# Jhuighuy/StormRuler

Measured on AMD Instinct MI355X. Metric: CG iterations/sec, 256^3 Poisson per GPU (+ SpMV achieved HBM GB/s in `roofline`), higher is better.
Workload: dtype f64

## Files before the change

stormruler_amd/csrc/common.hpp:

```cpp
#pragma once

#include <hip/hip_runtime.h>

#include <cstdint>
#include <cstdio>
#include <string>
#include <unordered_map>
#include <vector>

#include "../../include/storm_hip.h"

namespace storm {

void set_error(const char *fmt, ...) __attribute__((format(printf, 1, 2)));

#define STORM_FAIL(code, ...)        \
  do {                               \
    ::storm::set_error(__VA_ARGS__); \
    return (code);                   \
  } while (0)

#define STORM_REQUIRE(cond, ...) \
  do {                           \
    if (!(cond)) STORM_FAIL(STORM_HIP_E_INVALID, __VA_ARGS__); \
// ... 95 lines not shown
    int k = 0;
    bool ready = false;
    double value[storm::kMaxMulti] = {};
  } result_ring[storm::kResultRing];
  storm::SolverState *d_state = nullptr;
  storm::SolverState *h_state = nullptr;
  unsigned long long *h_done_ring = nullptr;
  unsigned long long *d_done_ring = nullptr;
  std::vector<storm::KrylovRes> krylov_free;
  unsigned long long ring_gen = 0;
  int64_t opt_ell_cap = 0;
  int64_t opt_spmv_dict = 4;
  int64_t opt_spmv_spw = 0;
  int64_t opt_spmv_xcd_remap = 8;
  int64_t opt_spmv_xcd_remap_sell = 64;
  int64_t opt_nt = 1;
  int stream_reverse = 0;
  int spmv_reverse = 0;
  int64_t opt_spmv_canon_tile_min_rows = (int64_t)1 << 20;
  int64_t opt_spmv_record_index = 1;
  int64_t opt_spmv_canon_tile = 2;
  int64_t opt_mgs_steps = 4;
  int64_t opt_resident_early = 1;
  int64_t opt_resident_apply_cache = 1;
  int64_t opt_resident_halo_interleave = 1;
  int64_t opt_coop_mgs_prefetch = 1;
  int64_t opt_coop_mgs_lds_prefetch = 1;
  int64_t opt_coop_mgs_rotate_early = 1;
  int64_t opt_coop_mgs_alternate = 1;
  int64_t opt_coop_mgs_xcd_runs = 1;
  int64_t opt_coop_mgs_apply = 1;
  int64_t opt_coop_mgs_quad = 1;
  char *d_quad_slots = nullptr;
  int64_t opt_coop_mgs_lds = 1;
  int64_t opt_spmv_mixed = 1;
  int64_t opt_profile_spmv = 0;
  std::vector<storm::LazyStmt> lazy_q;
  std::unordered_map<const void *, int> occupancy;
  int64_t opt_test_disable = 0;
  int64_t opt_lazy = 0;
  int callback_depth = 0;
  int64_t n_lazy_fused_dots = 0, n_lazy_fused_pairs = 0, n_lazy_apply_dots = 0, n_lazy_cg_steps = 0;
  storm_hip_vec *lazy_spare = nullptr;
  int64_t opt_profile_comm = 0;
  int64_t opt_blas1_nt = 1;
  int64_t opt_coop_mgs = 1;
  int64_t opt_latency_publish = 1;
  int64_t opt_coop_plain = 1;
  int64_t opt_coop_force_fail = 0;
  int coop_ran = 0;
  int coop_disabled = 0;
  int coop_fallback = 0;
  int64_t coop_skip = 0, coop_backoff = 0;
  int64_t opt_latency_path = 1;
  int64_t opt_resident_path = 1;
  int64_t opt_resident_max_rows = (int64_t)1 << 22;
  int64_t opt_resident_planes = 0;
  char *d_res_exch = nullptr;
  int64_t res_exch_rows = 0;
  int64_t opt_resident_profile = 0;
  long long *d_res_prof = nullptr;
  int res_prof_blocks = 0;
  char *d_res_slots = nullptr;
  int opt_lin_fuse = 1;
  int64_t opt_ticket_verify_inject = 0;
  int64_t opt_ticket_verify = 0;
  int opt_ticket_reduce = 1;
  int opt_fused_reduce = 1;
  int opt_latency_cache = 1;
  int64_t opt_latency_rows = 1 << 19;
  int64_t opt_rccl_fused = 1;
  int64_t opt_rccl_ticket = 1;
  int64_t opt_comm_wait_seconds = 120;
  int64_t opt_rccl_flag_wait = 1;
  int64_t opt_rccl_early_halo = 1;
  int64_t opt_generic_solvers = 0;
  int64_t opt_cg_march_fill = 2048;
  int64_t opt_cg_march_alternate = 1;
  int64_t opt_cg_march = 8;
  int64_t opt_cg_residual_march = 1;
  int64_t opt_cg_residual_planes = 1;
  int64_t opt_cg_residual_chunk = 16;
  int64_t opt_cg_residual_fill = 512;
  int64_t opt_cg_fuse = 1;
  std::vector<std::pair<size_t, double *>> pool;
  struct VecArena {
    char *base = nullptr;
    size_t bytes = 0, pitch = 0;
    int slots = 0, used = 0;
  };
  std::vector<VecArena> arenas;
  int64_t opt_vec_arena = 1;
  size_t pool_bytes = 0;
  int64_t opt_pool_bytes = (int64_t)16 << 30;
  std::vector<hipEvent_t> prof_events;
  size_t prof_used = 0;
  const int *api_done = nullptr;
  int64_t n_resident_solves = 0, n_latency_solves = 0, n_throughput_solves = 0, n_engine_solves = 0, n_cg_fused_steps = 0;
  int64_t n_block_solves = 0;
  int64_t n_cg_residual_marches = 0;
  int64_t n_cg_residual_plane_marches = 0;
  int64_t n_mgs_chain_steps = 0, n_mgs_quad_steps = 0;
  storm::Comm *comm = nullptr;
  int n_ranks = 1, rank = 0;
};

struct storm_hip_vec {
  storm_hip_ctx *ctx = nullptr;
  int64_t n_owned = 0, n_halo = 0;
  double *d = nullptr;
  double *base = nullptr;
  size_t bytes = 0;
  bool exposed = false;
};
constexpr int kVecGuard = 32;

namespace storm {

struct HaloPlan {
  int n_nbrs = 0;
  std::vector<int> nbr_rank;
  std::vector<int64_t> send_ptr, recv_ptr;
  int *d_send_idx = nullptr;
  double *d_sendbuf = nullptr;
  int64_t n_send = 0;
};

}

struct storm_hip_op {
  storm_hip_ctx *ctx = nullptr;
  int64_t n_rows = 0, n_halo = 0;
  int64_t n_slices = 0, n_interior_slices = 0;
  int64_t nnz = 0, ell_slots = 0, max_row_len = 0;
  int64_t *d_slice_off = nullptr;
  char *d_pack = nullptr;
  double *d_dict = nullptr;
  int dict_size = 0;
  int *d_offs = nullptr;
  int offs_size = 0;
  int xcd_group_sell = 0;
  int pair = 0;
  uint8_t *d_rec_idx = nullptr;
  uint64_t *d_rec_words = nullptr;
  int rec_words = 0;
  char *d_bnd_pack = nullptr;
  int bnd_width = 0;
  int canon_k = 0, canon_m1 = -1;
  int canon_off[7] = {0, 0, 0, 0, 0, 0, 0};
  int64_t pack_bytes = 0;
  int64_t spw = 1;
  int64_t tail_rows = 0, tail_nnz = 0;
  int *d_tail_row = nullptr;
  int64_t *d_tail_ptr = nullptr;
  int *d_tail_col = nullptr;
  double *d_tail_val = nullptr;
  int uniform_width = 0;
  std::vector<int> h_interior, h_boundary;
  int *d_interior = nullptr, *d_boundary = nullptr;
  int64_t n_interior = 0, n_boundary = 0;
  int64_t int_plane0 = 0, int_plane1 = 0;
  int64_t device_bytes = 0;
  char *d_lat_pack = nullptr;
  int64_t *d_lat_off = nullptr;
  int64_t lat_bytes = 0;
  storm::HaloPlan halo;
};

namespace storm {

struct Scal {
  const double *p;
  double v;
  double sign;
};
static inline Scal host_scal(double v) { return Scal{nullptr, v, 1.0}; }
static inline Scal dev_scal(const double *p, double sign = 1.0) { return Scal{p, 0.0, sign}; }

constexpr int kUnroll = 4;
constexpr int kStreamBlockElems = kBlock * kUnroll * 2;
constexpr int kMaxStreamBlocks = 32768;
static inline int stream_blocks(int64_t n) {
  int64_t b = (n + kStreamBlockElems - 1) / kStreamBlockElems;
  if (b < 1) b = 1;
// ... 136 lines not shown
```

stormruler_amd/csrc/context.hip:

```cpp
#include <cstdarg>
#include <cstring>
#include <random>

#include <algorithm>
#include "common.hpp"

#include <cstddef>

namespace storm {

static thread_local char g_error[1024] = "";

void set_error(const char *fmt, ...) {
  va_list ap;
  va_start(ap, fmt);
  vsnprintf(g_error, sizeof g_error, fmt, ap);
  va_end(ap);
}

}

using namespace storm;

static void pool_release(storm_hip_ctx *c);
// ... 110 lines not shown
    strncpy(name, c->name.c_str(), (size_t)name_len - 1);
    name[name_len - 1] = 0;
  }
  if (num_cus) *num_cus = c->num_cus;
  if (total_mem_bytes) *total_mem_bytes = c->total_mem;
  return STORM_HIP_OK;
}

int storm_hip_ctx_set_option(storm_hip_ctx *c, const char *key, int64_t value) {
  STORM_REQUIRE(c && key, "ctx_set_option: null argument");
  if (!strcmp(key, "ell_cap")) c->opt_ell_cap = value;
  else if (!strcmp(key, "generic_solvers")) c->opt_generic_solvers = value;
  else if (!strcmp(key, "rccl_fused")) c->opt_rccl_fused = value;
  else if (!strcmp(key, "rccl_ticket")) c->opt_rccl_ticket = value;
  else if (!strcmp(key, "rccl_early_halo")) c->opt_rccl_early_halo = value;
  else if (!strcmp(key, "rccl_flag_wait")) c->opt_rccl_flag_wait = value;
  else if (!strcmp(key, "comm_wait_seconds")) {
    STORM_REQUIRE(value >= 1 && value <= 3600, "ctx_set_option: comm_wait_seconds %lld (1 .. 3600)", (long long)value);
    c->opt_comm_wait_seconds = value;
  }
  else if (!strcmp(key, "latency_path")) c->opt_latency_path = value;
  else if (!strcmp(key, "resident_path")) c->opt_resident_path = value;
  else if (!strcmp(key, "resident_max_rows")) c->opt_resident_max_rows = value;
  else if (!strcmp(key, "resident_planes")) c->opt_resident_planes = value;
  else if (!strcmp(key, "resident_profile")) c->opt_resident_profile = value;
  else if (!strcmp(key, "coop_force_fail")) c->opt_coop_force_fail = value;
  else if (!strcmp(key, "coop_mgs")) c->opt_coop_mgs = value;
  else if (!strcmp(key, "coop_mgs_lds")) c->opt_coop_mgs_lds = value;
  else if (!strcmp(key, "coop_mgs_quad")) c->opt_coop_mgs_quad = value;
  else if (!strcmp(key, "cg_march_fill")) c->opt_cg_march_fill = value;
  else if (!strcmp(key, "resident_early")) c->opt_resident_early = value;
  else if (!strcmp(key, "mgs_steps")) c->opt_mgs_steps = value;
  else if (!strcmp(key, "vec_arena")) c->opt_vec_arena = value;
  else if (!strcmp(key, "spmv_mixed")) c->opt_spmv_mixed = value;
  else if (!strcmp(key, "spmv_canon_tile")) c->opt_spmv_canon_tile = value;
  else if (!strcmp(key, "spmv_canon_tile_min_rows")) c->opt_spmv_canon_tile_min_rows = value;
  else if (!strcmp(key, "fused_reduce")) c->opt_fused_reduce = (int)value;
  else if (!strcmp(key, "ticket_reduce")) c->opt_ticket_reduce = (int)value;
  else if (!strcmp(key, "ticket_verify")) c->opt_ticket_verify = value;
  else if (!strcmp(key, "ticket_verify_inject")) c->opt_ticket_verify_inject = value;
  else if (!strcmp(key, "lin_fuse")) c->opt_lin_fuse = (int)value;
  else if (!strcmp(key, "latency_rows")) c->opt_latency_rows = value;
  else if (!strcmp(key, "latency_cache")) c->opt_latency_cache = (int)value;
  else if (!strcmp(key, "nontemporal")) c->opt_nt = value;
  else if (!strcmp(key, "spmv_dict")) c->opt_spmv_dict = value;
  else if (!strcmp(key, "pool_bytes")) {
    c->opt_pool_bytes = value;
    if ((int64_t)c->pool_bytes > value || (value == 0 && !c->pool.empty())) {
      (void)hipStreamSynchronize(c->stream);
      pool_release(c);
    }
  }
  else if (!strcmp(key, "spmv_spw")) c->opt_spmv_spw = value;
  else if (!strcmp(key, "spmv_xcd_remap")) {
    STORM_REQUIRE(value >= 0 && value <= 4096, "ctx_set_option: spmv_xcd_remap %lld (0 .. 4096)", (long long)value);
    c->opt_spmv_xcd_remap = c->opt_spmv_xcd_remap_sell = value;
  }
  else if (!strcmp(key, "test_disable")) {
    c->opt_test_disable = value;
    c->opt_coop_mgs_apply = !(value & 1), c->opt_coop_mgs_prefetch = c->opt_coop_mgs_lds_prefetch = !(value & 2);
    c->opt_resident_apply_cache = !(value & 4), c->opt_resident_halo_interleave = !(value & 8);
    c->opt_latency_publish = !(value & 16), c->opt_coop_plain = !(value & 32), c->opt_cg_march_alternate = !(value & 64);
    c->opt_coop_mgs_xcd_runs = !(value & 128), c->opt_coop_mgs_alternate = !(value & 256);
    c->opt_coop_mgs_rotate_early = !(value & 512);
  }
  else if (!strcmp(key, "lazy_statements")) {
    if (value == 0) {
      STORM_TRY(lazy_sync(c));
      if (c->lazy_spare) (void)storm_hip_vec_destroy(c->lazy_spare), c->lazy_spare = nullptr;
    }
    c->opt_lazy = value;
  }
  else if (!strcmp(key, "profile_spmv")) c->opt_profile_spmv = value;
  else if (!strcmp(key, "profile_comm")) {
    c->opt_profile_comm = value;
    if (value != 0) STORM_TRY(comm_profile_reset(c));
  }
  else if (!strcmp(key, "cg_fuse")) c->opt_cg_fuse = value;
  else if (!strcmp(key, "cg_march")) c->opt_cg_march = value;
  else if (!strcmp(key, "cg_residual_march")) c->opt_cg_residual_march = value;
  else if (!strcmp(key, "cg_residual_planes")) c->opt_cg_residual_planes = value;
  else if (!strcmp(key, "cg_residual_chunk")) c->opt_cg_residual_chunk = value;
  else if (!strcmp(key, "cg_residual_fill")) c->opt_cg_residual_fill = value;
  else if (!strcmp(key, "spmv_record_index")) c->opt_spmv_record_index = value;
  else if (!strcmp(key, "blas1_nt")) c->opt_blas1_nt = value;
  else STORM_FAIL(STORM_HIP_E_INVALID, "ctx_set_option: unknown key '%s'", key);
  return STORM_HIP_OK;
}

int storm_hip_ctx_get_counter(storm_hip_ctx *c, const char *key, int64_t *value) {
  STORM_REQUIRE(c && key && value, "ctx_get_counter: null argument");
  if (!strcmp(key, "resident_solves")) *value = c->n_resident_solves;
  else if (!strcmp(key, "latency_solves")) *value = c->n_latency_solves;
  else if (!strcmp(key, "throughput_solves")) *value = c->n_throughput_solves;
  else if (!strcmp(key, "engine_solves")) *value = c->n_engine_solves;
  else if (!strcmp(key, "block_solves")) *value = c->n_block_solves;
  else if (!strcmp(key, "cg_fused_steps")) *value = c->n_cg_fused_steps;
  else if (!strcmp(key, "cg_residual_marches")) *value = c->n_cg_residual_marches;
  else if (!strcmp(key, "cg_residual_plane_marches")) *value = c->n_cg_residual_plane_marches;
  else if (!strcmp(key, "mgs_chain_steps")) *value = c->n_mgs_chain_steps;
  else if (!strcmp(key, "mgs_quad_steps")) *value = c->n_mgs_quad_steps;
  else if (!strcmp(key, "lazy_fused_dots")) *value = c->n_lazy_fused_dots;
  else if (!strcmp(key, "lazy_fused_pairs")) *value = c->n_lazy_fused_pairs;
  else if (!strcmp(key, "lazy_apply_dots")) *value = c->n_lazy_apply_dots;
  else if (!strcmp(key, "lazy_cg_steps")) *value = c->n_lazy_cg_steps;
  else if (!strcmp(key, "lazy_waiting")) *value = (int64_t)c->lazy_q.size();
  else if (!strncmp(key, "ipc_", 4)) {
    static const char *names[6] = {"ipc_allreduce_wait_ticks", "ipc_allreduces", "ipc_ack_wait_ticks", "ipc_ack_waits",
                                   "ipc_halo_slow_poll_ticks", "ipc_halo_slow_polls"};
    int k = -1;
    for (int i = 0; i < 6; ++i)
      if (!strcmp(key, names[i])) k = i;
    STORM_REQUIRE(k >= 0, "ctx_get_counter: unknown key '%s'", key);
    const long long v = comm_ipc_stat(c, k);
    STORM_REQUIRE(v >= 0, "ctx_get_counter: '%s' needs the peer-window transport", key);
    *value = v;
  }
  else if (!strncmp(key, "rccl_prof_", 10)) {
    static const char *names[8] = {"rccl_prof_exchanges", "rccl_prof_event_to_comm_ticks", "rccl_prof_pack_ticks",
                                   "rccl_prof_sendrecv_ticks", "rccl_prof_unhidden_wait_ticks", "rccl_prof_resume_ticks",
                                   "rccl_prof_allreduces", "rccl_prof_allreduce_ticks"};
    int k = -1;
    for (int i = 0; i < 8; ++i)
      if (!strcmp(key, names[i])) k = i;
    STORM_REQUIRE(k >= 0, "ctx_get_counter: unknown key '%s'", key);
    const long long v = comm_profile_read(c, k);
    STORM_REQUIRE(v >= 0, "ctx_get_counter: '%s' needs the RCCL transport with option profile_comm = 1", key);
    *value = v;
  }
  else if (!strncmp(key, "resident_phase_max_", 19) || !strncmp(key, "resident_phase_mean_", 20)) {
    const bool mx = key[15] == 'm' && key[16] == 'a';
    const int k = atoi(key + (mx ? 19 : 20));
    STORM_REQUIRE(c->d_res_prof != nullptr && c->res_prof_blocks > 0 && k >= 0 && k < 8, "ctx_get_counter: no resident profile (option resident_profile)");
    std::vector<long long> h((size_t)c->res_prof_blocks * 8);
    HIP_TRY(hipStreamSynchronize(c->stream));
    HIP_TRY(hipMemcpy(h.data(), c->d_res_prof, sizeof(long long) * h.size(), hipMemcpyDeviceToHost));
    long long m = 0, sum = 0;
    for (int b = 0; b < c->res_prof_blocks; ++b) m = std::max(m, h[(size_t)b * 8 + k]), sum += h[(size_t)b * 8 + k];
    *value = mx ? m : sum / c->res_prof_blocks;
  } else if (!strncmp(key, "resident_phase_block_", 21)) {
    int b = 0, k = 0;
    STORM_REQUIRE(sscanf(key + 21, "%d_%d", &b, &k) == 2 && c->d_res_prof != nullptr && b >= 0 && b < c->res_prof_blocks && k >= 0 && k < 8,
                  "ctx_get_counter: no such block / phase");
    long long v = 0;
    HIP_TRY(hipStreamSynchronize(c->stream));
    HIP_TRY(hipMemcpy(&v, c->d_res_prof + (size_t)b * 8 + k, sizeof v, hipMemcpyDeviceToHost));
    *value = v;
  }
  else STORM_FAIL(STORM_HIP_E_INVALID, "ctx_get_counter: unknown key '%s'", key);
  return STORM_HIP_OK;
}

int storm_hip_ctx_get_spmv_profile(storm_hip_ctx *c, int64_t *launches, double *total_ms, double *min_ms) {
  STORM_REQUIRE(c, "get_spmv_profile: null context");
  HIP_TRY(hipStreamSynchronize(c->stream));
  double total = 0.0, mn = 0.0;
  const size_t pairs = c->prof_used / 2;
  for (size_t i = 0; i < pairs; ++i) {
    float ms = 0.f;
    HIP_TRY(hipEventElapsedTime(&ms, c->prof_events[2 * i], c->prof_events[2 * i + 1]));
    total += ms;
    if (i == 0 || ms < mn) mn = ms;
  }
  if (launches) *launches = (int64_t)pairs;
  if (total_ms) *total_ms = total;
  if (min_ms) *min_ms = mn;
  c->prof_used = 0;
  return STORM_HIP_OK;
}

int storm_hip_ctx_get_spmv_profile_samples(storm_hip_ctx *c, double *ms_out, int64_t capacity, int64_t *count) {
  STORM_REQUIRE(c && count && (ms_out || capacity == 0), "get_spmv_profile_samples: null argument");
  HIP_TRY(hipStreamSynchronize(c->stream));
  const size_t pairs = c->prof_used / 2;
  for (size_t i = 0; i < pairs && (int64_t)i < capacity; ++i) {
    float ms = 0.f;
    HIP_TRY(hipEventElapsedTime(&ms, c->prof_events[2 * i], c->prof_events[2 * i + 1]));
    ms_out[i] = ms;
  }
  *count = (int64_t)pairs;
  c->prof_used = 0;
  return STORM_HIP_OK;
// ... 354 lines not shown
```

stormruler_amd/csrc/solver_cg.hip:

```cpp
#include <algorithm>
#include "solver_fused.hpp"
#include "blas1_device.hpp"
#include "spmv_device.hpp"

namespace storm {

__device__ __forceinline__ double cg_r_alpha(SolverState *st, const double *__restrict__ pz_partials, int n_pz, double *lds4) {
  double pz;
  if (pz_partials) {
    pz = block_fold(pz_partials, n_pz, lds4);
    if (blockIdx.x == 0 && threadIdx.x == 0) st->s[S_PZ] = pz;
  } else {
    pz = st->s[S_PZ];
  }
  const double alpha = safe_divide(st->s[S_GAMMA], pz);
  if (blockIdx.x == 0 && threadIdx.x == 0) st->s[S_ALPHA] = alpha;
  return alpha;
}
__device__ __forceinline__ void cg_r_finish(SolverState *st, double acc, unsigned bx, double *__restrict__ partials,
                                            const TicketArgs &tickets, const IpcDev &w, int use_ipc, double *lds4) {
  const double s = block_sum256(acc, lds4);
  if (tickets.cnt == nullptr) {
    if (threadIdx.x == 0) partials[bx] = s;
    return;
  }
  if (threadIdx.x >= kWave) return;
  const double mine[1] = {s};
  double total[1];
  if (ticket_reduce_wave0<1>(tickets, mine, 1, bx, gridDim.x, total)) {
    if (use_ipc == 1) ipc_allreduce_wave<1>(w, total, 1);
    if (threadIdx.x == 0) {
      st->s[S_GAMMA_NEW] = total[0];
      if (use_ipc != 2) do_step(STEP_CG_RR, st, GmresDev{});
    }
  }
}

__global__ __launch_bounds__(kBlock) void cg_r_kernel(int64_t n, SolverState *st, double *__restrict__ r,
                                                      const double *__restrict__ z,
                                                      double *__restrict__ partials, int nt,
                                                      const double *__restrict__ pz_partials, int n_pz, int reverse,
                                                      TicketArgs tickets, IpcDev w, int use_ipc) {
  if (st->done) return;
  __shared__ double lds4[4];
  const unsigned bx = reverse ? gridDim.x - 1 - blockIdx.x : blockIdx.x;
  const double alpha = cg_r_alpha(st, pz_partials, n_pz, lds4);
  double acc = 0.0;
  const int64_t n2 = n >> 1;
  double2v *r2 = reinterpret_cast<double2v *>(r);
  const double2v *z2 = reinterpret_cast<const double2v *>(z);
  nt_dispatch(nt, [&](auto nt) {
  for (int64_t base = (int64_t)bx * (kBlock * kUnroll) + threadIdx.x; base < n2;
       base += (int64_t)gridDim.x * (kBlock * kUnroll)) {
    double2v vr[kUnroll], vz[kUnroll];
#pragma unroll
    for (int u = 0; u < kUnroll; ++u) {
      const int64_t i = base + u * kBlock;
      if (i < n2) vr[u] = ldv(r2 + i, nt), vz[u] = ldv(z2 + i, nt);
    }
#pragma unroll
    for (int u = 0; u < kUnroll; ++u) {
      const int64_t i = base + u * kBlock;
      if (i < n2) {
        vr[u] -= alpha * vz[u];
        stv(r2 + i, vr[u], nt);
        acc += vr[u].x * vr[u].x;
        acc += vr[u].y * vr[u].y;
      }
    }
  }
  });
  if ((n & 1) && bx == 0 && threadIdx.x == 0) {
    const double vr = r[n - 1] - alpha * z[n - 1];
    r[n - 1] = vr;
    acc += vr * vr;
  }
  cg_r_finish(st, acc, bx, partials, tickets, w, use_ipc, lds4);
}

template <bool IDX>
__global__ __launch_bounds__(kBlock) void cg_r_recompute_kernel(int64_t n, SolverState *st, double *__restrict__ r,
                                                                const double *__restrict__ p, SellArgs A, CanonTileArgs T,
                                                                Scal alpha_s, Scal beta_s, const double *__restrict__ pz_partials,
                                                                int n_pz, int reverse, TicketArgs tickets) {
  if (st->done) return;
  __shared__ double lds4[4];
  __shared__ double dict_sh[32];
  extern __shared__ __attribute__((aligned(16))) unsigned long long words_sh[];
  const int lane = threadIdx.x & (kWave - 1);
  if (threadIdx.x < 32) dict_sh[threadIdx.x] = A.dict[threadIdx.x];
  if (IDX) rec_table_fill(A, words_sh);
  __syncthreads();
  const unsigned bx = reverse ? gridDim.x - 1 - blockIdx.x : blockIdx.x;
  const double alpha = cg_r_alpha(st, pz_partials, n_pz, lds4);
  const double op_alpha = ld_scal2(alpha_s), op_beta = ld_scal2(beta_s);
  const int64_t a = T.a, b = T.b, mg = T.max_gather;
  const char *pg = reinterpret_cast<const char *>(p) - (size_t)kVecGuard * 8;
  auto pair_at = [&](int64_t row) {
    int64_t gi = row + kVecGuard;
    gi = gi < 0 ? 0 : (gi > mg ? mg : gi);
// ... 8 lines not shown
  const int64_t n2 = n >> 1;
  double2v *r2 = reinterpret_cast<double2v *>(r);
  for (int64_t base = (int64_t)bx * (kBlock * kUnroll) + threadIdx.x; base - lane < n2;
       base += (int64_t)gridDim.x * (kBlock * kUnroll)) {
    double2v vr[kUnroll], c[kUnroll], nb[kUnroll][4];
    double el[kUnroll];
    RecRaw<IDX> w[kUnroll];
#pragma unroll
    for (int u = 0; u < kUnroll; ++u) {
      const int64_t i = base + u * kBlock;
      const int64_t row = 2 * (i < n2 ? i : n2 - 1);
      vr[u] = r2[row >> 1];
      c[u] = pair_at(row);
      w[u] = rec_load<IDX>(A, (uint32_t)row);
      nb[u][0] = pair_at(row - b), nb[u][1] = pair_at(row - a), nb[u][2] = pair_at(row + a), nb[u][3] = pair_at(row + b);
      el[u] = 0.0;
      if (lane == 0) el[u] = one_at(row - 1);
      if (lane == kWave - 1) el[u] = one_at(row + 2);
    }
#pragma unroll
    for (int u = 0; u < kUnroll; ++u) {
      const int64_t i = base + u * kBlock;
      double2v xg[6];
      xg[0] = nb[u][0], xg[1] = nb[u][1], xg[4] = nb[u][2], xg[5] = nb[u][3];
      const double left = dpp_shift<0x138>(c[u].y);
      const double right = dpp_shift<0x130>(c[u].x);
      xg[2].x = lane == 0 ? el[u] : left;
      xg[2].y = c[u].x;
      xg[3].x = c[u].y;
      xg[3].y = lane == kWave - 1 ? el[u] : right;
      const double2v vz = lattice_pair_apply(dict_sh, rec_word<IDX>(w[u], words_sh), xg, c[u], op_alpha, op_beta);
      if (i < n2) {
        vr[u] -= alpha * vz;
        r2[i] = vr[u];
        acc += vr[u].x * vr[u].x;
        acc += vr[u].y * vr[u].y;
      }
    }
  }
  cg_r_finish(st, acc, bx, nullptr, tickets, IpcDev{}, 0, lds4);
}

static bool cg_r_recompute_applies(const storm_hip_op *op, bool tick) {
  storm_hip_ctx *c = op->ctx;
  MarchArgs M;
  int nb = 0;
  return c->opt_cg_residual_march != 0 && tick && c->comm == nullptr && c->opt_ticket_verify == 0 && op->n_rows % 2 == 0 &&
         spmv_can_march(op) && cg_march_geometry(op, &M, &nb);
}
static int cg_r_recompute_run(const storm_hip_op *op, int nbv, Scal alpha, Scal beta, const double *p, SolverState *st, double *r,
                              const double *pz_partials, int n_pz, int reverse) {
  storm_hip_ctx *c = op->ctx;
  CanonTileArgs T;
  int nbt = 0;
  STORM_REQUIRE(canon_tile_geometry(op, &T, &nbt), "cg: the residual recompute needs a lattice operator");
  const SellArgs A = lattice_args(op);
  const size_t lds = sizeof(uint64_t) * (size_t)A.rec_words_n;
  const TicketArgs tk{c->d_tickets, c->d_partials, c->d_ticket_sums};
  if (A.rec_idx != nullptr)
    hipLaunchKernelGGL(cg_r_recompute_kernel<true>, dim3(nbv), dim3(kBlock), lds, c->stream, op->n_rows, st, r, p, A, T, alpha,
                       beta, pz_partials, n_pz, reverse, tk);
  else
    hipLaunchKernelGGL(cg_r_recompute_kernel<false>, dim3(nbv), dim3(kBlock), lds, c->stream, op->n_rows, st, r, p, A, T, alpha,
                       beta, pz_partials, n_pz, reverse, tk);
  HIP_TRY(hipGetLastError());
  return STORM_HIP_OK;
}

struct ResidualPlanesArgs {
  int a, b;
  int runs_per_plane;
  int per_xcd;
  int planes;
  int nz;
  int max_gather;
};
constexpr int kResidualMaxChunk = 32;
template <int HLP, bool IDX>
__global__ __launch_bounds__(kBlock) void cg_r_planes_kernel(SolverState *st, double *__restrict__ r, const double *__restrict__ p,
                                                             SellArgs A, ResidualPlanesArgs G, Scal alpha_s, Scal beta_s,
                                                             const double *__restrict__ pz_partials, int n_pz, int reverse,
                                                             TicketArgs tickets) {
  const int done = st->done;
  __shared__ double lds4[4];
  __shared__ double dict_sh[32];
  __shared__ double wave_part[kResidualMaxChunk * (kBlock / kWave)];
  extern __shared__ __attribute__((aligned(16))) double plane_sh[];
  const int a = G.a, b = G.b;
  const int ldw = kStreamBlockElems + 2 * a;
  unsigned long long *words_sh = reinterpret_cast<unsigned long long *>(plane_sh + 2 * ldw);
  const int lane = threadIdx.x & (kWave - 1);
  const int wave = __builtin_amdgcn_readfirstlane(threadIdx.x >> 6);
  const int bidx = reverse ? (int)(gridDim.x - 1 - blockIdx.x) : (int)blockIdx.x;
  int zc, yt;
  if (G.per_xcd > 0) {
    const int xcd = bidx & (kNumXcd - 1), j = bidx >> 3;
    zc = j / G.per_xcd;
    yt = xcd * G.per_xcd + (j - zc * G.per_xcd);
  } else {
    zc = bidx / G.runs_per_plane;
    yt = bidx - zc * G.runs_per_plane;
  }
  const int z_begin = zc * G.nz, z_end = min(z_begin + G.nz, G.planes), nz = z_end - z_begin;
  auto plane = [&](int s) { return z_begin + s; };
  const int p0 = yt * kStreamBlockElems;
  const char *pg = reinterpret_cast<const char *>(p) - (size_t)kVecGuard * 8;
  double2v *r2 = reinterpret_cast<double2v *>(r);

  struct Flight {
    double2v p[kUnroll], hp[HLP];
  };
  int hat[HLP], hjj[HLP];
#pragma unroll
  for (int i = 0; i < HLP; ++i) {
    const int h = (int)threadIdx.x + kBlock * i;
    hjj[i] = 2 * h < a ? 2 * h - a : kStreamBlockElems + 2 * h - a;
    hat[i] = h < a ? a + hjj[i] : -1;
  }
  auto load_p = [&](int64_t row) {
    int64_t gi = row + kVecGuard;
    gi = gi < 0 ? 0 : (gi > (int64_t)G.max_gather ? (int64_t)G.max_gather : gi);
    return *reinterpret_cast<const double2v *>(pg + (size_t)gi * 8);
  };
  auto issue_p = [&](int zp, bool own, Flight &f) {
    const int64_t row0 = (int64_t)zp * b + p0;
#pragma unroll
    for (int u = 0; u < kUnroll; ++u) f.p[u] = load_p(row0 + 2 * ((int)threadIdx.x + kBlock * u));
#pragma unroll
    for (int i = 0; i < HLP; ++i) {
      f.hp[i] = double2v{0.0, 0.0};
      if (own && hat[i] >= 0) f.hp[i] = load_p(row0 + hjj[i]);
    }
  };
  auto issue_rw = [&](int zp, double2v (&vr)[kUnroll], RecRaw<IDX> (&w)[kUnroll]) {
    const int64_t row0 = (int64_t)zp * b + p0;
#pragma unroll
    for (int u = 0; u < kUnroll; ++u) {
      const int64_t row = row0 + 2 * ((int)threadIdx.x + kBlock * u);
      vr[u] = r2[row >> 1];
      w[u] = rec_load<IDX>(A, (uint32_t)row);
    }
  };

  Flight cur, nxt, fl;
  double2v pm[kUnroll], vr[kUnroll];
  RecRaw<IDX> w[kUnroll];
  issue_p(plane(-1), false, fl);
#pragma unroll
  for (int u = 0; u < kUnroll; ++u) pm[u] = fl.p[u];
  issue_p(plane(0), true, cur);
  issue_rw(plane(0), vr, w);
  issue_p(plane(1), 1 < nz, nxt);
  if (threadIdx.x < 32) dict_sh[threadIdx.x] = A.dict[threadIdx.x];
  if (IDX) rec_table_fill(A, words_sh);
  if (done) return;
  const double alpha = cg_r_alpha(st, pz_partials, n_pz, lds4);
  const double op_alpha = ld_scal2(alpha_s), op_beta = ld_scal2(beta_s);
  for (int s = 0; s < nz; ++s) {
    const int zp = plane(s);
    double *buf = plane_sh + (s & 1) * ldw;
#pragma unroll
    for (int u = 0; u < kUnroll; ++u) *reinterpret_cast<double2v *>(&buf[a + 2 * ((int)threadIdx.x + kBlock * u)]) = cur.p[u];
#pragma unroll
    for (int i = 0; i < HLP; ++i)
      if (hat[i] >= 0) *reinterpret_cast<double2v *>(&buf[hat[i]]) = cur.hp[i];
    double2v vrn[kUnroll];
    RecRaw<IDX> wn[kUnroll];
    if (s + 2 <= nz) issue_p(plane(s + 2), s + 2 < nz, fl);
    if (s + 1 < nz) issue_rw(plane(s + 1), vrn, wn);
    __syncthreads();
    const int64_t i0 = (((int64_t)zp * b + p0) >> 1) + threadIdx.x;
    double acc = 0.0;
#pragma unroll
    for (int u = 0; u < kUnroll; ++u) {
      const int at = a + 2 * ((int)threadIdx.x + kBlock * u);
      double2v xg[6];
      march_neighbours(buf, at, a, lane, pm[u], nxt.p[u], cur.p[u], xg);
      const double2v vz = lattice_pair_apply(dict_sh, rec_word<IDX>(w[u], words_sh), xg, cur.p[u], op_alpha, op_beta);
      vr[u] -= alpha * vz;
      r2[i0 + u * kBlock] = vr[u];
      acc += vr[u].x * vr[u].x;
      acc += vr[u].y * vr[u].y;
    }
    acc = wave_sum_down(acc);
    if (lane == 0) wave_part[s * (kBlock / kWave) + wave] = acc;
#pragma unroll
    for (int u = 0; u < kUnroll; ++u) pm[u] = cur.p[u], vr[u] = vrn[u], w[u] = wn[u];
    cur = nxt, nxt = fl;
  }
  __syncthreads();
  if (threadIdx.x >= kWave) return;
  const bool on = lane < nz;
  const double mine = on ? block_sum256_of_waves(wave_part + lane * (kBlock / kWave)) : 0.0;
  const unsigned bxv = on ? (unsigned)(plane(lane) * G.runs_per_plane + yt) : 0u;
  double total;
  if (ticket_reduce_wave0_slots(tickets, mine, on, bxv, (unsigned)(G.planes * G.runs_per_plane), &total) && threadIdx.x == 0) {
    st->s[S_GAMMA_NEW] = total;
    do_step(STEP_CG_RR, st, GmresDev{});
  }
}

static bool cg_r_planes_geometry(const storm_hip_op *op, ResidualPlanesArgs *G, int *n_blocks) {
  storm_hip_ctx *c = op->ctx;
  CanonTileArgs T;
  int nbt = 0;
  if (c->opt_cg_residual_planes == 0 || !canon_tile_geometry(op, &T, &nbt)) return false;
  const int64_t n = op->n_rows;
  if (T.b % kStreamBlockElems != 0 || n % T.b != 0 || n / kStreamBlockElems > kMaxStreamBlocks) return false;
  if ((int64_t)sizeof(double) * 2 * (kStreamBlockElems + 2 * T.a) + (int64_t)sizeof(uint64_t) * op->rec_words > 60 * 1024) return false;
  G->a = T.a, G->b = T.b, G->max_gather = T.max_gather;
  G->runs_per_plane = T.b / kStreamBlockElems;
  G->per_xcd = (G->runs_per_plane % kNumXcd == 0 && c->opt_spmv_xcd_remap != 0) ? G->runs_per_plane / kNumXcd : 0;
  G->planes = (int)(n / T.b);
  const int64_t zc = std::min<int64_t>(std::max<int64_t>(c->opt_cg_residual_chunk, 2), kResidualMaxChunk);
  const int64_t want = c->opt_cg_residual_fill;
  const int64_t fill = want > 0 ? (int64_t)G->planes * G->runs_per_plane / want : zc;
  G->nz = (int)std::min<int64_t>(std::min<int64_t>(zc, std::max<int64_t>(2, fill)), G->planes);
  *n_blocks = ((G->planes + G->nz - 1) / G->nz) * G->runs_per_plane;
  return true;
}
static int cg_r_planes_run(const storm_hip_op *op, const ResidualPlanesArgs &G, int n_blocks, Scal alpha, Scal beta, const double *p,
                           SolverState *st, double *r, const double *pz_partials, int n_pz, int reverse) {
  storm_hip_ctx *c = op->ctx;
  const SellArgs A = lattice_args(op);
  const size_t lds = sizeof(double) * 2 * (size_t)(kStreamBlockElems + 2 * G.a) + sizeof(uint64_t) * (size_t)A.rec_words_n;
  const TicketArgs tk{c->d_tickets, c->d_partials, c->d_ticket_sums};
#define PLANES_GO(HLP_, IX_)                                                                                                   \
  hipLaunchKernelGGL((cg_r_planes_kernel<HLP_, IX_>), dim3(n_blocks), dim3(kBlock), lds, c->stream, st, r, p, A, G, alpha, beta, \
                     pz_partials, n_pz, reverse, tk)
  if (G.a <= kBlock) {
    if (A.rec_idx != nullptr) PLANES_GO(1, true);
    else PLANES_GO(1, false);
  } else {
    if (A.rec_idx != nullptr) PLANES_GO(2, true);
    else PLANES_GO(2, false);
  }
#undef PLANES_GO
  HIP_TRY(hipGetLastError());
  return STORM_HIP_OK;
}

constexpr int kUnrollXp = 1;
__global__ __launch_bounds__(kBlock) void cg_xp_kernel(int64_t n, const SolverState *st, long long my_iteration,
                                                       double *__restrict__ x, double *__restrict__ p,
                                                       const double *__restrict__ r, int nt, int reverse) {
  if (st->iteration < my_iteration) return;
  const unsigned bx = reverse ? gridDim.x - 1 - blockIdx.x : blockIdx.x;
  const bool update_p = !st->done && r != nullptr;
  const double alpha = st->s[S_ALPHA], beta = st->s[S_BETA];
  const int64_t n2 = n >> 1;
  double2v *x2 = reinterpret_cast<double2v *>(x), *p2 = reinterpret_cast<double2v *>(p);
  const double2v *r2 = reinterpret_cast<const double2v *>(r);
  nt_dispatch(nt, [&](auto nt) {
  for (int64_t base = (int64_t)bx * (kBlock * kUnrollXp) + threadIdx.x; base < n2;
       base += (int64_t)gridDim.x * (kBlock * kUnrollXp)) {
    double2v vx[kUnrollXp], vp[kUnrollXp], vr[kUnrollXp];
#pragma unroll
    for (int u = 0; u < kUnrollXp; ++u) {
      const int64_t i = base + u * kBlock;
      if (i < n2) {
        vx[u] = ldv(x2 + i, nt), vp[u] = ldv(p2 + i, nt);
        if (update_p) vr[u] = ldv(r2 + i, nt);
      }
    }
#pragma unroll
    for (int u = 0; u < kUnrollXp; ++u) {
      const int64_t i = base + u * kBlock;
      if (i < n2) {
        vx[u] += alpha * vp[u];
        stv(x2 + i, vx[u], nt);
        if (update_p) stv(p2 + i, vr[u] + beta * vp[u], nt);
      }
    }
  }
  });
  if ((n & 1) && bx == 0 && threadIdx.x == 0) {
    const int64_t i = n - 1;
    x[i] += alpha * p[i];
    if (update_p) p[i] = r[i] + beta * p[i];
  }
}
static inline int xp_blocks(int64_t n) {
  int64_t b = ((n >> 1) + kBlock * kUnrollXp - 1) / (kBlock * kUnrollXp);
  return (int)(b < 1 ? 1 : (b > 131072 ? 131072 : b));
}


struct CgRoads {
  bool may_fuse_step;
  bool ipc, tick;
  bool tick_spmv;
  bool rccl, fuse_step;
  bool rtick;
  bool r_march;
  bool r_planes;
  ResidualPlanesArgs planes_args;
  int planes_blocks = 0;
};
static CgRoads cg_roads(Driver &d, int nbv) {
  storm_hip_ctx *c = d.c;
  CgRoads w;
  w.may_fuse_step = c->opt_cg_fuse != 0 && spmv_can_fuse_cg(d.op);
  w.ipc = c->comm != nullptr && comm_ipc_next(c, &d.ipc_w);
  w.tick = c->opt_ticket_reduce != 0 && (c->comm == nullptr || w.ipc) && nbv <= kTicketGroup * kTicketMaxGroups;
  w.tick_spmv = w.tick && !w.ipc && 4 * (int64_t)spmv_grid_blocks(d.op) <= kSinglePassPartials;
  w.rccl = c->comm != nullptr && comm_is_rccl(c);
  w.fuse_step = w.may_fuse_step && (w.rccl ? true : ((c->comm == nullptr || w.ipc) && w.tick && !w.tick_spmv));
  w.rtick = w.rccl && w.fuse_step && c->opt_ticket_reduce != 0 && c->opt_rccl_ticket != 0 && nbv <= kTicketGroup * kTicketMaxGroups;
  w.r_march = w.fuse_step && !w.rccl && cg_r_recompute_applies(d.op, w.tick);
  w.r_planes = w.r_march && cg_r_planes_geometry(d.op, &w.planes_args, &w.planes_blocks);
  if (w.fuse_step) ++c->n_cg_fused_steps;
  if (w.r_march) ++c->n_cg_residual_marches;
  if (w.r_planes) ++c->n_cg_residual_plane_marches;
  return w;
}

static int solve_cg_body(const FusedSolveArgs &args) {
  const storm_hip_op *op = args.op;
  const double *b = args.b->d;
  double *x = args.x->d;
  Driver d;
  STORM_TRY(prepare_state(args, &d));
  storm_hip_ctx *c = d.c;
  const int64_t n = d.n;
  VecPool pool;
  if (res_eligible(op, false)) {
    bool taken = false;
    STORM_TRY(res_solve(false, op, d.alpha, d.beta, b, x, nullptr, c->d_state, &taken));
    if (taken) return ++c->n_resident_solves, collect(d, args, 1);
  }
  if (cg_latency_eligible(op)) {
    STORM_TRY(pool.make(args.x, 2));
    bool taken = false;
    STORM_TRY(cg_latency_solve(op, d.alpha, d.beta, b, x, pool.v[0]->d, pool.v[1]->d, c->d_state, &taken));
    if (taken) return ++c->n_latency_solves, collect(d, args, 1);
  }
  ++c->n_throughput_solves;
  const size_t v0 = pool.v.size();
  const int nbv = stream_blocks(n);
  const CgRoads road = cg_roads(d, nbv);
  STORM_TRY(pool.make(args.x, road.may_fuse_step ? 4 : 3, false));
  static const int kRolesFused[4] = {1, 2, 0, 3}, kRolesPlain[3] = {0, 1, 2};
  const int *role = road.may_fuse_step ? kRolesFused : kRolesPlain;
  double *p = pool.v[v0 + role[0]]->d, *r = pool.v[v0 + role[1]]->d, *z = pool.v[v0 + role[2]]->d;
  double *p_alt = road.fuse_step ? pool.v[v0 + role[3]]->d : nullptr;

  int nb = 0;
  STORM_TRY(d.apply(x, r, &nb, {}, false));
  STORM_TRY(d.init_residual(r, b, p));
  STORM_TRY(d.finish(nbv, 1, S_GAMMA, STEP_CG_INIT, true));
  int64_t cur_it = 0;
  const int nt_stream = stream_nt(c, n);
  int64_t last_enqueued = -1;
  auto enqueue_iteration = [&]() -> int {
    const int q = road.fuse_step ? 0 : (int)(cur_it & 1);
    c->spmv_reverse = q;
    int pz_done = 0;
    int st_apply;
    const bool r_march_now = road.r_march && cur_it > 0;
    if (road.fuse_step && cur_it > 0) {
      const CgStep step{(long long)cur_it, x, r, p_alt};
      st_apply = d.apply(p, r_march_now ? nullptr : z, &nb, {.w = p, .ticketed = &pz_done}, true, &step);
      std::swap(p, p_alt);
    } else {
      st_apply = d.apply(p, z, &nb, {.w = p, .out0 = road.tick_spmv ? (int)S_PZ : -1, .ticketed = &pz_done});
    }
    last_enqueued = cur_it;
    c->spmv_reverse = 0;
    STORM_TRY(st_apply);
    const bool tickets_now = road.tick && (nb > kSinglePassPartials || road.ipc);
    const Driver::Road allow = road.rtick ? Driver::ROAD_TICKETS_RCCL
                                          : !tickets_now ? Driver::ROAD_PLAIN : road.ipc ? Driver::ROAD_TICKETS_IPC : Driver::ROAD_TICKETS;
    Driver::Road ran;
    const double *pz_partials = nullptr, *const pz_with[1] = {z};
    STORM_TRY(d.finish_dots(pz_done, nb, 1, S_PZ, p, pz_with, allow, STEP_NONE, &ran, &pz_partials));
    if (r_march_now && road.r_planes) {
      STORM_TRY(cg_r_planes_run(op, road.planes_args, road.planes_blocks, host_scal(d.alpha), host_scal(d.beta), p, d.st, r, pz_partials,
                                (int)kStage2, 1 - q));
    } else if (r_march_now) {
      STORM_TRY(cg_r_recompute_run(op, nbv, host_scal(d.alpha), host_scal(d.beta), p, d.st, r, pz_partials, (int)kStage2, 1 - q));
    } else {
      hipLaunchKernelGGL(cg_r_kernel, dim3(nbv), dim3(kBlock), 0, c->stream, n, d.st, r, z, c->d_partials, nt_stream, pz_partials,
                         (int)kStage2, 1 - q, (road.tick || road.rtick) ? d.tickets() : TicketArgs{}, d.ipc_w,
                         road.rtick ? 2 : (int)(road.ipc && road.tick));
      HIP_TRY(hipGetLastError());
    }
    if (road.rtick) {
      STORM_TRY(comm_allreduce_sum(c, d.slot(S_GAMMA_NEW), 1));
      STORM_TRY(d.step(STEP_CG_RR));
    } else if (!road.tick) {
      STORM_TRY(d.finish(nbv, 1, S_GAMMA_NEW, STEP_CG_RR));
    }
    if (road.tick && c->opt_ticket_verify > 0 && cur_it % c->opt_ticket_verify == 0) {
      STORM_TRY(d.verify(p, z, nullptr, S_PZ, -1, (long long)(cur_it + 1)));
      STORM_TRY(d.verify(r, r, nullptr, S_GAMMA, -1, (long long)(cur_it + 1)));
    }
    if (road.fuse_step) return STORM_HIP_OK;
    if (road.rccl && c->opt_rccl_early_halo != 0 && op->halo.n_nbrs > 0)
      STORM_TRY(comm_halo_exchange_begin_formed(op, 2, r, p, nullptr, d.slot(S_BETA), nullptr, p));
    hipLaunchKernelGGL(cg_xp_kernel, dim3(xp_blocks(n)), dim3(kBlock), 0, c->stream, n, d.st, (long long)(cur_it + 1), x, p, r,
                       nt_stream, q);
    HIP_TRY(hipGetLastError());
    return STORM_HIP_OK;
  };
  for (int64_t it = 0; it < args.params->num_iterations; ++it) {
    cur_it = it;
    STORM_TRY(enqueue_iteration());
    bool stop = false;
    STORM_TRY(post_and_poll(d, it, &stop));
    if (stop) break;
  }
  if (road.fuse_step && last_enqueued >= 0) {
    hipLaunchKernelGGL(cg_xp_kernel, dim3(xp_blocks(n)), dim3(kBlock), 0, c->stream, n, d.st, (long long)(last_enqueued + 1), x, p,
                       (const double *)nullptr, nt_stream, 0);
    HIP_TRY(hipGetLastError());
  }
  comm_forget_prebegun(c);
  return collect(d, args, 1);
}

}

extern "C" int storm_hip_solve_cg(const storm_hip_op *op, double alpha, double beta, const storm_hip_vec *b, storm_hip_vec *x,
                                  const storm_hip_solver_params *params, storm_hip_solver_result *result, double *history) {
  if (op) STORM_TRY(storm::lazy_sync(op->ctx));
  return storm::fused_solve(storm::FusedSolveArgs{op, alpha, beta, b, x, params, result, history, &storm::solve_cg_body});
}
```

stormruler_amd/csrc/solver_device.hpp:

```cpp
#pragma once

#include "common.hpp"
#include "ipc_device.hpp"
#include "wave_device.hpp"

namespace storm {

__device__ __forceinline__ double safe_divide(double x, double y) { return (y == 0.0) ? 0.0 : (x / y); }

__device__ inline void advance(SolverState *st, double abs_err) {
  st->absolute_error = abs_err;
  st->relative_error = abs_err / st->initial_error;
  bool conv = false;
  conv |= (st->abs_tol > 0.0) && (st->absolute_error < st->abs_tol);
  conv |= (st->rel_tol > 0.0) && (st->relative_error < st->rel_tol);
  st->iteration += 1;
  if (st->history) st->history[st->iteration] = abs_err;
  if (conv) st->converged = 1;
  if (conv || st->iteration >= st->num_iterations) st->done = 1;
  if (st->done_ring)
    __hip_atomic_store(st->done_ring + (st->iteration - 1) % kStateRing,
                       ring_word(st->ring_gen, (unsigned long long)st->iteration, st->done != 0), __ATOMIC_RELAXED,
                       __HIP_MEMORY_SCOPE_SYSTEM);
}

__device__ inline void begin(SolverState *st, double initial_error) {
  st->initial_error = initial_error;
  st->absolute_error = initial_error;
  st->relative_error = 0.0;
  st->iteration = 0;
  st->converged = 0;
  st->done = 0;
  if (st->history) st->history[0] = initial_error;
  if (st->abs_tol > 0.0 && initial_error < st->abs_tol) st->converged = 1, st->done = 1;
  if (st->num_iterations <= 0) st->done = 1;
  if (st->done && st->done_ring)
    for (int i = 0; i < kStateRing; ++i)
      __hip_atomic_store(st->done_ring + i, ring_word(st->ring_gen, kRingIterMask, true), __ATOMIC_RELAXED, __HIP_MEMORY_SCOPE_SYSTEM);
}

struct GmresDev {
  double *H, *beta, *cs, *sn;
  int m;
};
__device__ inline void gmres_givens_update(SolverState *st, GmresDev g, int k, double hn) {
  const int m = g.m;
#define H_(i, j) g.H[(i) * m + (j)]
  H_(k + 1, k) = hn;
  for (int i = 0; i < k; ++i) {
    const double chi = g.cs[i] * H_(i, k) + g.sn[i] * H_(i + 1, k);
    H_(i + 1, k) = -g.sn[i] * H_(i, k) + g.cs[i] * H_(i + 1, k);
    H_(i, k) = chi;
  }
  const double a = H_(k, k), b = H_(k + 1, k);
  const double rr = hypot(a, b);
  double cs, sn;
  if (rr > 0.0) cs = a / rr, sn = b / rr;
  else cs = 1.0, sn = 0.0;
  g.cs[k] = cs, g.sn[k] = sn;
  H_(k, k) = cs * H_(k, k) + sn * H_(k + 1, k);
  H_(k + 1, k) = 0.0;
  g.beta[k + 1] = -sn * g.beta[k];
  g.beta[k] *= cs;
  advance(st, fabs(g.beta[k + 1]));
#undef H_
}

__device__ __forceinline__ double block_sum256_of_waves(const double *lds4) { return (lds4[0] + lds4[1]) + (lds4[2] + lds4[3]); }
__device__ __forceinline__ double block_sum256(double v, double *lds4) {
  v = wave_sum_down(v);
  const int lane = threadIdx.x & (kWave - 1), wave = threadIdx.x >> 6;
  __syncthreads();
  if (lane == 0) lds4[wave] = v;
  __syncthreads();
  return block_sum256_of_waves(lds4);
}

__device__ __forceinline__ double block_fold(const double *__restrict__ p, int i0, int i1, double *lds4) {
  double v = 0.0;
#pragma unroll 8
  for (int i = i0 + threadIdx.x; i < i1; i += kBlock) v += p[i];
  return block_sum256(v, lds4);
}
__device__ __forceinline__ double block_fold(const double *__restrict__ p, int n, double *lds4) {
  return block_fold(p, 0, n, lds4);
}

template <int K>
struct OutPtrs {
  double *p[K];
};

template <class Epi, int K>
__global__ __launch_bounds__(kBlock) void reduce_finish_kernel(const double *__restrict__ partials, int nblocks, int k,
                                                               OutPtrs<K> out, const int *done, IpcDev w, int use_ipc, Epi epi) {
  if (done && *done) return;
  __shared__ double lds4[4];
  __shared__ double vals[K];
  for (int j = 0; j < k; ++j) {
    const double sum = block_fold(partials + (int64_t)j * nblocks, nblocks, lds4);
    if (threadIdx.x == 0) vals[j] = sum;
  }
  if (use_ipc) ipc_allreduce_block(w, vals, k);
  else __syncthreads();
  if ((int)threadIdx.x < k) *out.p[threadIdx.x] = vals[threadIdx.x];
  __syncthreads();
  if (threadIdx.x == 0) epi();
}

template <class Epi, int K, class Tail>
int k_reduce_finish(storm_hip_ctx *c, const double *partials, int nblocks, int k, const OutPtrs<K> &out, const int *done,
                    const Epi &epi, const OutPtrs<K> &local, Tail rccl_tail) {
  STORM_TRY(k_reduce_stage1(c, &partials, &nblocks, k, done));
  IpcDev w{};
  const bool one = c->comm == nullptr || comm_ipc_next(c, &w);
  hipLaunchKernelGGL((reduce_finish_kernel<Epi, K>), dim3(1), dim3(kBlock), 0, c->stream, partials, nblocks, k, one ? out : local,
                     done, w, (int)(c->comm != nullptr && one), one ? epi : Epi{});
  HIP_TRY(hipGetLastError());
  return one ? STORM_HIP_OK : rccl_tail();
}

}
```

Measured before the change: 5379.

## Fold <p,z> partials inside the residual plane march instead of a separate finish

When the residual plane march runs single-rank without tickets, the <p,z> block partials are no longer reduced by a separate finish_dots launch. The march kernel issues the partial loads early, overlaps them with its plane prefetch, and folds them itself to compute alpha. The r·r partials are moved to a separate offset in the partials buffer so the two do not collide. block_fold is also restructured to issue batched loads, and there is a capacity check on the partials count. This saves a kernel launch and a dependency per iteration, but every block redundantly folds up to kSinglePassPartials values and holds them in registers.

```diff
diff --git a/stormruler_amd/csrc/common.hpp b/stormruler_amd/csrc/common.hpp
--- a/stormruler_amd/csrc/common.hpp
+++ b/stormruler_amd/csrc/common.hpp
@@ -201,6 +201,7 @@
   int64_t opt_cg_residual_planes = 1;
   int64_t opt_cg_residual_chunk = 16;
   int64_t opt_cg_residual_fill = 512;
+  int64_t opt_cg_pz_fold = 1;
   int64_t opt_cg_fuse = 1;
   std::vector<std::pair<size_t, double *>> pool;
   struct VecArena {
@@ -219,6 +220,7 @@
   int64_t n_block_solves = 0;
   int64_t n_cg_residual_marches = 0;
   int64_t n_cg_residual_plane_marches = 0;
+  int64_t n_cg_pz_consumer_folds = 0;
   int64_t n_mgs_chain_steps = 0, n_mgs_quad_steps = 0;
   storm::Comm *comm = nullptr;
   int n_ranks = 1, rank = 0;
diff --git a/stormruler_amd/csrc/context.hip b/stormruler_amd/csrc/context.hip
--- a/stormruler_amd/csrc/context.hip
+++ b/stormruler_amd/csrc/context.hip
@@ -216,6 +216,7 @@
   else if (!strcmp(key, "cg_residual_planes")) c->opt_cg_residual_planes = value;
   else if (!strcmp(key, "cg_residual_chunk")) c->opt_cg_residual_chunk = value;
   else if (!strcmp(key, "cg_residual_fill")) c->opt_cg_residual_fill = value;
+  else if (!strcmp(key, "cg_pz_fold")) c->opt_cg_pz_fold = value;
   else if (!strcmp(key, "spmv_record_index")) c->opt_spmv_record_index = value;
   else if (!strcmp(key, "blas1_nt")) c->opt_blas1_nt = value;
   else STORM_FAIL(STORM_HIP_E_INVALID, "ctx_set_option: unknown key '%s'", key);
@@ -232,6 +233,7 @@
   else if (!strcmp(key, "cg_fused_steps")) *value = c->n_cg_fused_steps;
   else if (!strcmp(key, "cg_residual_marches")) *value = c->n_cg_residual_marches;
   else if (!strcmp(key, "cg_residual_plane_marches")) *value = c->n_cg_residual_plane_marches;
+  else if (!strcmp(key, "cg_pz_consumer_folds")) *value = c->n_cg_pz_consumer_folds;
   else if (!strcmp(key, "mgs_chain_steps")) *value = c->n_mgs_chain_steps;
   else if (!strcmp(key, "mgs_quad_steps")) *value = c->n_mgs_quad_steps;
   else if (!strcmp(key, "lazy_fused_dots")) *value = c->n_lazy_fused_dots;
diff --git a/stormruler_amd/csrc/solver_cg.hip b/stormruler_amd/csrc/solver_cg.hip
--- a/stormruler_amd/csrc/solver_cg.hip
+++ b/stormruler_amd/csrc/solver_cg.hip
@@ -5,17 +5,25 @@
 
 namespace storm {
 
-__device__ __forceinline__ double cg_r_alpha(SolverState *st, const double *__restrict__ pz_partials, int n_pz, double *lds4) {
+template <class Fold, class Gamma>
+__device__ __forceinline__ double cg_r_alpha_of(SolverState *st, bool folds, Fold fold, Gamma gamma) {
   double pz;
-  if (pz_partials) {
-    pz = block_fold(pz_partials, n_pz, lds4);
+  if (folds) {
+    pz = fold();
     if (blockIdx.x == 0 && threadIdx.x == 0) st->s[S_PZ] = pz;
   } else {
     pz = st->s[S_PZ];
   }
-  const double alpha = safe_divide(st->s[S_GAMMA], pz);
+  const double alpha = safe_divide(gamma(), pz);
   if (blockIdx.x == 0 && threadIdx.x == 0) st->s[S_ALPHA] = alpha;
   return alpha;
+}
+__device__ __forceinline__ double cg_r_alpha(SolverState *st, const double *__restrict__ pz_partials, int n_pz, double *lds4) {
+  return cg_r_alpha_of(st, pz_partials != nullptr, [&] { return block_fold(pz_partials, n_pz, lds4); }, [&] { return st->s[S_GAMMA]; });
+}
+__device__ __forceinline__ double cg_r_alpha(SolverState *st, bool folds, const FoldWhole &pz_flight, int n_pz, double gamma,
+                                             double *lds4) {
+  return cg_r_alpha_of(st, folds, [&] { return block_fold_sum(pz_flight, n_pz, lds4); }, [&] { return gamma; });
 }
 __device__ __forceinline__ void cg_r_finish(SolverState *st, double acc, unsigned bx, double *__restrict__ partials,
                                             const TicketArgs &tickets, const IpcDev &w, int use_ipc, double *lds4) {
@@ -190,6 +198,7 @@
                                                              const double *__restrict__ pz_partials, int n_pz, int reverse,
                                                              TicketArgs tickets) {
   const int done = st->done;
+  const double gamma = st->s[S_GAMMA];
   __shared__ double lds4[4];
   __shared__ double dict_sh[32];
   __shared__ double wave_part[kResidualMaxChunk * (kBlock / kWave)];
@@ -259,10 +268,13 @@
   issue_p(plane(0), true, cur);
   issue_rw(plane(0), vr, w);
   issue_p(plane(1), 1 < nz, nxt);
+  const bool folds = pz_partials != nullptr;
+  FoldWhole pz_flight;
+  if (folds) block_fold_issue(pz_partials, n_pz, pz_flight);
   if (threadIdx.x < 32) dict_sh[threadIdx.x] = A.dict[threadIdx.x];
   if (IDX) rec_table_fill(A, words_sh);
   if (done) return;
-  const double alpha = cg_r_alpha(st, pz_partials, n_pz, lds4);
+  const double alpha = cg_r_alpha(st, folds, pz_flight, n_pz, gamma, lds4);
   const double op_alpha = ld_scal2(alpha_s), op_beta = ld_scal2(beta_s);
   for (int s = 0; s < nz; ++s) {
     const int zp = plane(s);
@@ -328,11 +340,13 @@
   return true;
 }
 static int cg_r_planes_run(const storm_hip_op *op, const ResidualPlanesArgs &G, int n_blocks, Scal alpha, Scal beta, const double *p,
-                           SolverState *st, double *r, const double *pz_partials, int n_pz, int reverse) {
+                           SolverState *st, double *r, const double *pz_partials, int n_pz, int reverse, double *rr_partials) {
   storm_hip_ctx *c = op->ctx;
+  STORM_REQUIRE(pz_partials == nullptr || n_pz <= kSinglePassPartials, "cg: the plane march folds at most %d partials of <p,z>, not %d",
+                kSinglePassPartials, n_pz);
   const SellArgs A = lattice_args(op);
   const size_t lds = sizeof(double) * 2 * (size_t)(kStreamBlockElems + 2 * G.a) + sizeof(uint64_t) * (size_t)A.rec_words_n;
-  const TicketArgs tk{c->d_tickets, c->d_partials, c->d_ticket_sums};
+  const TicketArgs tk{c->d_tickets, rr_partials, c->d_ticket_sums};
 #define PLANES_GO(HLP_, IX_)                                                                                                   \
   hipLaunchKernelGGL((cg_r_planes_kernel<HLP_, IX_>), dim3(n_blocks), dim3(kBlock), lds, c->stream, st, r, p, A, G, alpha, beta, \
                      pz_partials, n_pz, reverse, tk)
@@ -460,6 +474,7 @@
   int64_t cur_it = 0;
   const int nt_stream = stream_nt(c, n);
   int64_t last_enqueued = -1;
+  bool pz_fold_counted = false;
   auto enqueue_iteration = [&]() -> int {
     const int q = road.fuse_step ? 0 : (int)(cur_it & 1);
     c->spmv_reverse = q;
@@ -481,10 +496,17 @@
                                           : !tickets_now ? Driver::ROAD_PLAIN : road.ipc ? Driver::ROAD_TICKETS_IPC : Driver::ROAD_TICKETS;
     Driver::Road ran;
     const double *pz_partials = nullptr, *const pz_with[1] = {z};
-    STORM_TRY(d.finish_dots(pz_done, nb, 1, S_PZ, p, pz_with, allow, STEP_NONE, &ran, &pz_partials));
-    if (r_march_now && road.r_planes) {
+    const int64_t rr_slots = road.r_planes ? (int64_t)road.planes_args.planes * road.planes_args.runs_per_plane : 0;
+    const bool pz_fold_now = c->opt_cg_pz_fold != 0 && r_march_now && road.r_planes && c->comm == nullptr && !tickets_now &&
+                             !pz_done && nb > 0 && nb <= kSinglePassPartials && nb + rr_slots <= c->partials_capacity;
+    if (pz_fold_now && !pz_fold_counted) ++c->n_cg_pz_consumer_folds, pz_fold_counted = true;
+    if (!pz_fold_now) STORM_TRY(d.finish_dots(pz_done, nb, 1, S_PZ, p, pz_with, allow, STEP_NONE, &ran, &pz_partials));
+    if (pz_fold_now) {
+      STORM_TRY(cg_r_planes_run(op, road.planes_args, road.planes_blocks, host_scal(d.alpha), host_scal(d.beta), p, d.st, r, c->d_partials,
+                                nb, 1 - q, c->d_partials + nb));
+    } else if (r_march_now && road.r_planes) {
       STORM_TRY(cg_r_planes_run(op, road.planes_args, road.planes_blocks, host_scal(d.alpha), host_scal(d.beta), p, d.st, r, pz_partials,
-                                (int)kStage2, 1 - q));
+                                (int)kStage2, 1 - q, c->d_partials));
     } else if (r_march_now) {
       STORM_TRY(cg_r_recompute_run(op, nbv, host_scal(d.alpha), host_scal(d.beta), p, d.st, r, pz_partials, (int)kStage2, 1 - q));
     } else {
diff --git a/stormruler_amd/csrc/solver_device.hpp b/stormruler_amd/csrc/solver_device.hpp
--- a/stormruler_amd/csrc/solver_device.hpp
+++ b/stormruler_amd/csrc/solver_device.hpp
@@ -76,14 +76,46 @@
   return block_sum256_of_waves(lds4);
 }
 
+template <int B>
+struct FoldFlight {
+  double v[B];
+};
+template <int B>
+__device__ __forceinline__ void fold_issue(const double *__restrict__ p, int i, int i1, FoldFlight<B> &f) {
+#pragma unroll
+  for (int j = 0; j < B; ++j) {
+    f.v[j] = 0.0;
+    if (i + kBlock * j < i1) f.v[j] = p[i + kBlock * j];
+  }
+}
+template <int B>
+__device__ __forceinline__ void fold_add(const FoldFlight<B> &f, int i, int i1, double &v) {
+#pragma unroll
+  for (int j = 0; j < B; ++j)
+    if (i + kBlock * j < i1) v += f.v[j];
+}
 __device__ __forceinline__ double block_fold(const double *__restrict__ p, int i0, int i1, double *lds4) {
   double v = 0.0;
-#pragma unroll 8
-  for (int i = i0 + threadIdx.x; i < i1; i += kBlock) v += p[i];
+  for (int i = i0 + threadIdx.x; i < i1; i += kBlock * 8) {
+    FoldFlight<8> f;
+    fold_issue(p, i, i1, f);
+    fold_add(f, i, i1, v);
+  }
   return block_sum256(v, lds4);
 }
 __device__ __forceinline__ double block_fold(const double *__restrict__ p, int n, double *lds4) {
   return block_fold(p, 0, n, lds4);
+}
+constexpr int kFoldWhole = kSinglePassPartials / kBlock;
+static_assert(kFoldWhole * kBlock == kSinglePassPartials, "a whole fold holds kSinglePassPartials / kBlock values per thread");
+using FoldWhole = FoldFlight<kFoldWhole>;
+__device__ __forceinline__ void block_fold_issue(const double *__restrict__ p, int n, FoldWhole &f) {
+  fold_issue(p, (int)threadIdx.x, n, f);
+}
+__device__ __forceinline__ double block_fold_sum(const FoldWhole &f, int n, double *lds4) {
+  double v = 0.0;
+  fold_add(f, (int)threadIdx.x, n, v);
+  return block_sum256(v, lds4);
 }
 
 template <int K>
```

After: 5461, median of 6. 1.02x the previous value.
